# winddori2002/DEX-TTS

Hardware: AMD Instinct MI355X
Metric: mel-frames/s at n_timesteps=50, 80-ch mel (sampler only); RTF (higher is better)
Workload: dtype bf16; 1 GPU; gedex_b1: gedex_lj B=1/GPU T=512 n_timesteps=50 (BASELINE.json configs[1]); global_batch=1, frames=512, hipgraph=False, parallelism=1 GPU

## Files before the change

dex_tts_amd/csrc/dex_api.hip:

```cpp
#include <hip/hip_runtime.h>
#include <cstdlib>

#include <cmath>
#include <cstdarg>
#include <atomic>
#include <cstdio>
#include <mutex>
#include <cstring>
#include <map>
#include <unordered_map>
#include <string_view>
#include <string>
#include <vector>

#include "../../include/dex_amd.h"
#include "kernels.h"
#include "weight_store.h"

using namespace dex;

namespace dex {
namespace {
const char* const KNOB_NAMES[] = {
    "DEX_CONV_STREAM", "DEX_CONV_PP", "DEX_CONV_SKIP_DEAD", "DEX_H_BF16", "DEX_ATTN_SEPARATE", "DEX_ATTN_Q64", "DEX_ATTN_Q64_TAIL", "DEX_ATTN_Q64_HALF", "DEX_DIT_XCDS", "DEX_ATTN_GENERIC", "DEX_RES2", "DEX_LP_INTER", "DEX_DIT_CHAIN",
    "DEX_DIT_CLUSTER", "DEX_DIT_CLUSTER_LOCAL", "DEX_ATTN_X_LP", "DEX_RES_X_LP", "DEX_CAT_LP", "DEX_XCD_MAP", "DEX_DEBUG_DROP_HANDOFF", "DEX_PATCH_FUSED",
    "DEX_CONV_DOWN", "DEX_CONVT_UP", "DEX_DEBUG_PLAN",
    "DEX_ATTN_SHARED_W8", "DEX_CONVT_MT", "DEX_CONVT_WGS", "DEX_CONV_DOWN_WGS", "DEX_CONV_REGW", "DEX_CONV_REGW_RES", "DEX_CONV_SMALL_MAX", "DEX_CONV_TH8",
    "DEX_CONV_W8", "DEX_DWCONV_CAP", "DEX_FINAL_CAP", "DEX_FIRST_CAP", "DEX_FIRST_MFMA", "DEX_GEMM_NWALK", "DEX_NWALK_SPLIT", "DEX_NWALK_BM", "DEX_POS_COL", "DEX_POS_COL_MIN",
    "DEX_POS_CT", "DEX_REGW_MIN_TILES", "DEX_REGW_WGS", "DEX_ROWCHAIN64", "DEX_ROWCHAIN64A", "DEX_TIV_CAP", "DEX_TV_CHAIN", "DEX_TIV_FOLD", "DEX_LINATTN_NSUB", "DEX_TV_FOLD", "DEX_OUT2_MIN", "DEX_NWALK_DMA",
    "DEX_LINATTN_HEADWAVES", "DEX_LINATTN_OUT2_HW", "DEX_CONV_ROUND1", "DEX_CONV_RESIDENT", "DEX_KVCTX_ROWS", "DEX_OUT2_ROWS"};
constexpr int N_KNOBS = (int)(sizeof(KNOB_NAMES) / sizeof(KNOB_NAMES[0]));
int knob_parse(const char* e) {
    if (!e) return KNOB_UNSET;
    char* end = nullptr;
    const long v = strtol(e, &end, 10);
    if (end == e) {
        static bool warned = false;
        if (!warned) { warned = true; fprintf(stderr, "libdexamd: ignoring a DEX_* knob whose value '%s' is not an integer\n", e); }
        return KNOB_UNSET;
    }
    return (int)v;
}
struct KnobSnapshot {
    int v[N_KNOBS];
    KnobSnapshot() { for (int i = 0; i < N_KNOBS; ++i) v[i] = knob_parse(getenv(KNOB_NAMES[i])); }
};
thread_local const KnobSnapshot* t_knobs = nullptr;
struct WsplitScope {
    bool prev;
    explicit WsplitScope(bool on) : prev(g_lp_wsplit) { g_lp_wsplit = on; }
    ~WsplitScope() { g_lp_wsplit = prev; }
};
struct KnobScope {
    const KnobSnapshot* prev;
    explicit KnobScope(const KnobSnapshot* k) : prev(t_knobs) { t_knobs = k; }
    ~KnobScope() { t_knobs = prev; }
};
}
static int knob_index(const char* name) {
    static const std::unordered_map<std::string_view, int> idx = [] {
        std::unordered_map<std::string_view, int> m;
        for (int i = 0; i < N_KNOBS; ++i) m.emplace(KNOB_NAMES[i], i);
        return m;
// ... 1878 lines not shown
```

dex_tts_amd/csrc/igemm_bf16.hip:

```cpp
#include "kernels.h"
#include <cstdlib>
#include "lp_util.h"
#include "kernels_lp.h"
#include "igemm_epilogue.h"

namespace dex {
namespace DEX_LP_NS {

typedef unsigned short u16;


template <int BN, int BK, bool PT, int AP, int RPP, int BP, bool ALP = false>
__device__ __forceinline__ void igemm_load_tile(const IGemmP& p, float4 (&fa)[AP][2], float (&fm)[AP], float (&fo)[AP], uint4& rb0, uint4& rb1,
#ifdef DEX_LP_WSPLIT
                                                uint4& rl0, uint4& rl1,
#endif
                                                int k0, bool live, int tk8, int trow,
                                                const int (&bh)[AP], const int (&bw)[AP], unsigned mvbits,
                                                const float* Ab, const float* mrow, int mws, const u16* Wb, int n0) {
    const int kthr = PT ? k0 + tk8 : k0;
    const int tap = kthr / p.Cin, c0 = kthr - tap * p.Cin + (PT ? 0 : tk8);
    const int kh = tap / p.KW, kw = tap - kh * p.KW;
#pragma unroll
    for (int j = 0; j < AP; ++j) {
// ... 257 lines not shown
                c.z = c.z * rstd * (1.f + sc1.z) + sh1.z; c.w = c.w * rstd * (1.f + sc1.w) + sh1.w;
            }
            const float m_ = mk[j];
            uint4 v;
            v.x = pack2_lp(a.x * m_, a.y * m_); v.y = pack2_lp(a.z * m_, a.w * m_);
            v.z = pack2_lp(c.x * m_, c.y * m_); v.w = pack2_lp(c.z * m_, c.w * m_);
            *reinterpret_cast<uint4*>(As + row * LDS_LD + k8) = v;
        }
    }
    __syncthreads();
    f32x16 acc[MT];
#pragma unroll
    for (int t = 0; t < MT; ++t)
#pragma unroll
        for (int r = 0; r < 16; ++r) acc[t][r] = 0.f;
    const u16* ap = As + (wm * (MT * 32) + i) * LDS_LD + hh * 8;
    const u16* bp = Bs + (wn * 32 + i) * LDS_LD + hh * 8;
#pragma unroll
    for (int ks = 0; ks < K / 16; ++ks) {
        const lp8 bf = *reinterpret_cast<const lp8*>(bp + ks * 16);
#pragma unroll
        for (int t = 0; t < MT; ++t) {
            const lp8 af = *reinterpret_cast<const lp8*>(ap + t * 32 * LDS_LD + ks * 16);
            acc[t] = DEX_MFMA_LP(af, bf, acc[t], 0, 0, 0);
#ifdef DEX_LP_WSPLIT
            acc[t] = DEX_MFMA_LP(af, __builtin_bit_cast(lp8, bl_[ks]), acc[t], 0, 0, 0);
#endif
        }
    }
    igemm_epilogue<MT>(p, acc, m0, n0, wm * (MT * 32), wn * 32, lane, b, 0, 0, M, oh0, ow0);
}

typedef unsigned u32x4 __attribute__((ext_vector_type(4)));
template <int K, int BM = 64, bool DMA = false>
__global__ __launch_bounds__(BM * 4) void igemm_lp_nwalk_kernel(const IGemmP p) {
    constexpr int BN = 64, NTHR = BM * 4;
    constexpr int WN = BN / 32, WM = BM / 32, MT = 1;
    constexpr int LDS_LD = K + 8, KC = K / 8;
    constexpr int AIT = BM * KC / NTHR, BIT = BN * KC / NTHR;
    constexpr int ABATCH = AIT > 8 ? 8 : AIT;
    constexpr int TILE = BN * K;
    static_assert(!DMA || BM == 64, "DMA form: 64-row workgroups");
    extern __shared__ __attribute__((aligned(16))) u16 smem_ss[];
    u16* As = DMA ? smem_ss + TILE : smem_ss;
    u16* Bs = smem_ss + BM * LDS_LD;
    typedef __attribute__((address_space(3))) void* lds_ptr_t;
    const int tid = threadIdx.x, lane = tid & 63, wave = tid >> 6;
    const int i = lane & 31, hh = lane >> 5;
    const int wm = wave / WN, wn = wave % WN;
    const int b = blockIdx.z;
    const int M = p.Ho * p.Wo;
    const int m0 = blockIdx.x * BM;
    const int ntile_all = p.N / BN;
    const int ntile = ntile_all / (int)gridDim.y, nt_first = blockIdx.y * ntile;
    const float* Ab = p.A + (long)b * p.a_bstride + p.a_coff;
    const float* mrow = p.inmask ? p.inmask + (long)b * p.mask_bstride : nullptr;
    const u16* Wb = reinterpret_cast<const u16*>(p.Wbf) + (long)b * p.w_bstride + (long)nt_first * BN * K;
    const int step = p.step + b * p.row_bstride;
    const float* lsh = p.ln_shift ? p.ln_shift + (long)step * p.ln_step_stride : nullptr;
    const float* lsc = p.ln_scale ? p.ln_scale + (long)step * p.ln_step_stride : nullptr;

    const u16* Wf = DMA ? reinterpret_cast<const u16*>(p.Wfrag) + (long)b * p.w_bstride + (long)nt_first * TILE : nullptr;
#define NW_DMA(nt_)                                                                                                 \
    _Pragma("unroll") for (int j = 0; j < 8; ++j) {                                                                \
        const int piece = 8 * wave + j;                                                                             \
        __builtin_amdgcn_global_load_lds(Wf + (long)(nt_) * TILE + piece * 512 + lane * 8,                          \
                                         (lds_ptr_t)(smem_ss + ((nt_) & 1) * TILE + piece * 512), 16, 0, 0);        \
    }
    float* sbias = reinterpret_cast<float*>(smem_ss + TILE + BM * LDS_LD);
    float* smk = sbias + p.N;
    if constexpr (DMA) {
        NW_DMA(0)
        const float* biasg = p.bias ? p.bias + (long)b * p.bias_bstride : nullptr;
        for (int idx = tid; idx < p.N; idx += NTHR) sbias[idx] = biasg ? biasg[idx] : 0.f;
        const float* omg = p.outmask ? p.outmask + (long)b * p.mask_bstride : nullptr;
        const int row = tid >> 2, mrow_ = m0 + row, mm_ = mrow_ < M ? mrow_ : 0, uw_ = (mm_ % p.Wo) * p.unpatch_s;
#pragma unroll
        for (int e = 0; e < 2; ++e) {
            const int sft = (tid & 3) + 4 * e;
            smk[row * 8 + sft] = omg ? omg[min(uw_ + sft, p.OWf - 1) * p.outmask_ws] : 1.f;
        }
    }
    u32x4 br[BIT];
#define NW_LOAD_B(nt_)                                                                                              \
    _Pragma("unroll") for (int j = 0; j < BIT; ++j) {                                                              \
        const int it = tid + NTHR * j;                                                                              \
        br[j] = *reinterpret_cast<const u32x4*>(Wb + (long)((nt_) * BN + it / KC) * K + (it % KC) * 8);            \
    }
#define NW_STORE_B()                                                                                                \
    _Pragma("unroll") for (int j = 0; j < BIT; ++j) {                                                              \
        const int it = tid + NTHR * j;                                                                              \
        *reinterpret_cast<u32x4*>(Bs + (it / KC) * LDS_LD + (it % KC) * 8) = br[j];                                 \
    }
#ifdef DEX_LP_WSPLIT
    const bool has_lo = p.w_lo_off != 0;
    u16* Bl = As;
    u32x4 brl[BIT];
#define NW_LOAD_LO(nt_)                                                                                             \
    _Pragma("unroll") for (int j = 0; j < BIT; ++j) {                                                              \
        const int it = tid + NTHR * j;                                                                              \
        const u32x4 v_ = *reinterpret_cast<const u32x4*>(Wb + (has_lo ? p.w_lo_off : 0) + (long)((nt_) * BN + it / KC) * K + (it % KC) * 8); \
        brl[j] = has_lo ? v_ : u32x4{0u, 0u, 0u, 0u};                                                               \
    }
#define NW_STORE_LO()                                                                                               \
    _Pragma("unroll") for (int j = 0; j < BIT; ++j) {                                                              \
        const int it = tid + NTHR * j;                                                                              \
        *reinterpret_cast<u32x4*>(Bl + (it / KC) * LDS_LD + (it % KC) * 8) = brl[j];                                \
    }
    NW_LOAD_LO(0)
#endif
    if constexpr (!DMA) { NW_LOAD_B(0) }
#pragma unroll
    for (int a0 = 0; a0 < AIT; a0 += ABATCH) {
        float4 f0[ABATCH], f1[ABATCH];
        float mk[ABATCH];
#pragma unroll
        for (int j = 0; j < ABATCH; ++j) {
            const int it = tid + NTHR * (a0 + j);
            const int row = it / KC, k8 = (it % KC) * 8;
            const int m = m0 + row;
            const int mm = m < M ? m : 0;
            const float* src = Ab + (long)mm * p.lda + k8;
            f0[j] = *reinterpret_cast<const float4*>(src);
            f1[j] = *reinterpret_cast<const float4*>(src + 4);
            const float mv = mrow ? mrow[(mm % p.Wi) * p.inmask_ws] : 1.f;
            mk[j] = m < M ? mv : 0.f;
        }
        if constexpr (!DMA) { if (a0 == 0) { NW_STORE_B() } }
#pragma unroll
        for (int j = 0; j < ABATCH; ++j) {
            const int it = tid + NTHR * (a0 + j);
            const int row = it / KC, k8 = (it % KC) * 8;
            float4 a = f0[j], c = f1[j];
            if (lsh) {
                float s = (a.x + a.y) + (a.z + a.w) + (c.x + c.y) + (c.z + c.w);
#pragma unroll
                for (int o = 1; o < KC; o <<= 1) s += __shfl_xor(s, o);
                const float mean = s * (1.f / (float)K);
                a.x -= mean; a.y -= mean; a.z -= mean; a.w -= mean; c.x -= mean; c.y -= mean; c.z -= mean; c.w -= mean;
                float q = a.x * a.x + a.y * a.y + a.z * a.z + a.w * a.w + c.x * c.x + c.y * c.y + c.z * c.z + c.w * c.w;
#pragma unroll
                for (int o = 1; o < KC; o <<= 1) q += __shfl_xor(q, o);
                const float rstd = rsqrtf(q * (1.f / (float)K) + 1e-6f);
                const float4 sc0 = *reinterpret_cast<const float4*>(lsc + k8), sc1 = *reinterpret_cast<const float4*>(lsc + k8 + 4);
                const float4 sh0 = *reinterpret_cast<const float4*>(lsh + k8), sh1 = *reinterpret_cast<const float4*>(lsh + k8 + 4);
                a.x = a.x * rstd * (1.f + sc0.x) + sh0.x; a.y = a.y * rstd * (1.f + sc0.y) + sh0.y;
                a.z = a.z * rstd * (1.f + sc0.z) + sh0.z; a.w = a.w * rstd * (1.f + sc0.w) + sh0.w;
                c.x = c.x * rstd * (1.f + sc1.x) + sh1.x; c.y = c.y * rstd * (1.f + sc1.y) + sh1.y;
                c.z = c.z * rstd * (1.f + sc1.z) + sh1.z; c.w = c.w * rstd * (1.f + sc1.w) + sh1.w;
            }
            const float m_ = mk[j];
            uint4 v;
            v.x = pack2_lp(a.x * m_, a.y * m_); v.y = pack2_lp(a.z * m_, a.w * m_);
            v.z = pack2_lp(c.x * m_, c.y * m_); v.w = pack2_lp(c.z * m_, c.w * m_);
            *reinterpret_cast<uint4*>(As + row * LDS_LD + k8) = v;
        }
    }
    __syncthreads();
    const u16* ap = As + (wm * (MT * 32) + i) * LDS_LD + hh * 8;
    const u16* bp = Bs + (wn * 32 + i) * LDS_LD + hh * 8;
    static_assert(MT == 1, "one 32-row tile per wave");
    lp8 afr[K / 16];
#pragma unroll
    for (int ks = 0; ks < K / 16; ++ks) afr[ks] = *reinterpret_cast<const lp8*>(ap + ks * 16);
#ifdef DEX_LP_WSPLIT
    __syncthreads();
    NW_STORE_LO()
    __syncthreads();
    const u16* blp = Bl + (wn * 32 + i) * LDS_LD + hh * 8;
#endif
    int u_pix, u_f, u_w;
    {
        const int m = m0 + wm * 32 + i;
        const bool v = m < M;
        const int mm = v ? m : 0;
        const int f = mm / p.Wo, w = mm - f * p.Wo;
        u_f = v ? f * p.unpatch_s : 0x40000000;
        u_w = w * p.unpatch_s;
        u_pix = f * p.unpatch_s * p.OWf + w * p.unpatch_s;
    }
    const float* omask = p.outmask ? p.outmask + (long)b * p.mask_bstride : nullptr;
    const float* biasb = p.bias ? p.bias + (long)b * p.bias_bstride : nullptr;
    float4 dst4[4]; char* d_ptr = nullptr; bool d_ok = false, d_all = false, d_have = false;
#define NW_FLUSH()                                                                                                  \
    if (d_have) {                                                                                                   \
        if (p.c_lp) {                                                                                               \
            u16* c_ = reinterpret_cast<u16*>(d_ptr);                                                                \
            if (d_all) { *reinterpret_cast<float4*>(c_) = dst4[0]; *reinterpret_cast<float4*>(c_ + 16) = dst4[1]; } \
            else if (d_ok) { *reinterpret_cast<float4*>(c_) = dst4[0]; *reinterpret_cast<float4*>(c_ + 16) = dst4[1]; } \
        } else {                                                                                                    \
            float* c_ = reinterpret_cast<float*>(d_ptr);                                                            \
// ... 12 lines not shown
#ifdef DEX_LP_WSPLIT
        if (nt + 1 < ntile) { NW_LOAD_LO(nt + 1) }
#endif
        const int ng0 = (nt_first + nt) * BN + wn * 32, pp = ng0 / p.unpatch_C;
        const int u_c0 = ng0 - pp * p.unpatch_C;
        const int u_p1 = pp / p.unpatch_s, u_p2 = pp - u_p1 * p.unpatch_s;
        float u_mk;
        float4 b4[4];
        if constexpr (DMA) {
            u_mk = smk[(wm * 32 + i) * 8 + u_p2];
#pragma unroll
            for (int q = 0; q < 4; ++q) b4[q] = *reinterpret_cast<const float4*>(sbias + ng0 + 8 * q + 4 * hh);
            if (nt + 1 < ntile) { NW_DMA(nt + 1) }
            NW_FLUSH()
        } else {
            u_mk = omask ? omask[min(u_w + u_p2, p.OWf - 1) * p.outmask_ws] : 1.f;
#pragma unroll
            for (int q = 0; q < 4; ++q) b4[q] = biasb ? *reinterpret_cast<const float4*>(biasb + ng0 + 8 * q + 4 * hh) : make_float4(0.f, 0.f, 0.f, 0.f);
        }
        __builtin_amdgcn_sched_barrier(0);
        f32x16 acc[MT];
#pragma unroll
        for (int t = 0; t < MT; ++t)
#pragma unroll
            for (int r = 0; r < 16; ++r) acc[t][r] = 0.f;
#pragma unroll
        for (int ks = 0; ks < K / 16; ++ks) {
            const lp8 bf = *reinterpret_cast<const lp8*>(bp + ks * (DMA ? 512 : 16));
            acc[0] = DEX_MFMA_LP(bf, afr[ks], acc[0], 0, 0, 0);
#ifdef DEX_LP_WSPLIT
            acc[0] = DEX_MFMA_LP(*reinterpret_cast<const lp8*>(blp + ks * 16), afr[ks], acc[0], 0, 0, 0);
#endif
        }
        {
            float val[16];
#pragma unroll
            for (int q = 0; q < 4; ++q) {
                val[4 * q + 0] = (acc[0][4 * q + 0] + b4[q].x) * u_mk; val[4 * q + 1] = (acc[0][4 * q + 1] + b4[q].y) * u_mk;
                val[4 * q + 2] = (acc[0][4 * q + 2] + b4[q].z) * u_mk; val[4 * q + 3] = (acc[0][4 * q + 3] + b4[q].w) * u_mk;
            }
            const bool ok = u_f + u_p1 < p.OHf && u_w + u_p2 < p.OWf;
            const long e0 = (long)b * p.c_bstride + p.c_coff + (long)(u_p1 * p.OWf + u_p2 + u_pix) * p.ldc + u_c0;
            __builtin_amdgcn_sched_barrier(0);
            if (p.c_lp) {
                typedef unsigned u32x2n __attribute__((ext_vector_type(2)));
                unsigned D[4][2];
#pragma unroll
                for (int q = 0; q < 4; ++q) { D[q][0] = pack2_lp(val[4 * q], val[4 * q + 1]); D[q][1] = pack2_lp(val[4 * q + 2], val[4 * q + 3]); }
                uint4 ch[2];
#pragma unroll
                for (int pr = 0; pr < 2; ++pr) {
                    const u32x2n s0 = __builtin_amdgcn_permlane32_swap(D[2 * pr][0], D[2 * pr + 1][0], false, false);
                    const u32x2n s1 = __builtin_amdgcn_permlane32_swap(D[2 * pr][1], D[2 * pr + 1][1], false, false);
                    ch[pr] = make_uint4(s0[0], s1[0], s0[1], s1[1]);
                }
                u16* cph = reinterpret_cast<u16*>(p.C) + e0 + 8 * hh;
                if constexpr (DMA) {
                    dst4[0] = __builtin_bit_cast(float4, ch[0]); dst4[1] = __builtin_bit_cast(float4, ch[1]);
                    d_ptr = reinterpret_cast<char*>(cph); d_ok = ok; d_all = __builtin_amdgcn_ballot_w64(!ok) == 0; d_have = true;
                } else
                if (__builtin_amdgcn_ballot_w64(!ok) == 0) {
                    *reinterpret_cast<uint4*>(cph) = ch[0];
                    *reinterpret_cast<uint4*>(cph + 16) = ch[1];
                } else if (ok) {
                    *reinterpret_cast<uint4*>(cph) = ch[0];
                    *reinterpret_cast<uint4*>(cph + 16) = ch[1];
                }
            } else {
                float* cp = p.C + e0 + 4 * hh;
                if constexpr (DMA) {
#pragma unroll
                    for (int q = 0; q < 4; ++q) dst4[q] = make_float4(val[4 * q], val[4 * q + 1], val[4 * q + 2], val[4 * q + 3]);
                    d_ptr = reinterpret_cast<char*>(cp); d_ok = ok; d_all = __builtin_amdgcn_ballot_w64(!ok) == 0; d_have = true;
                } else
                if (__builtin_amdgcn_ballot_w64(!ok) == 0) {
#pragma unroll
                    for (int q = 0; q < 4; ++q) *reinterpret_cast<float4*>(cp + 8 * q) = make_float4(val[4 * q], val[4 * q + 1], val[4 * q + 2], val[4 * q + 3]);
                } else if (ok) {
#pragma unroll
                    for (int q = 0; q < 4; ++q) *reinterpret_cast<float4*>(cp + 8 * q) = make_float4(val[4 * q], val[4 * q + 1], val[4 * q + 2], val[4 * q + 3]);
                }
            }
        }
        if (!DMA && nt + 1 < ntile) {
            __syncthreads();
            NW_STORE_B()
#ifdef DEX_LP_WSPLIT
            NW_STORE_LO()
#endif
            __syncthreads();
        }
    }
    if constexpr (DMA) { NW_FLUSH() }
}

static bool nwalk_eligible(const IGemmP& p) {
    if (p.a_lp || p.act_in_slope != 0.f) return false;
    if (p.K != 256 || p.Cin != 256 || p.KH != 1 || p.KW != 1 || p.parity || p.ksplit != 1 || p.groups != 1 || (p.N % 64) != 0) return false;
    if (p.sh != 1 || p.sw != 1 || p.off_h != 0 || p.off_w != 0 || p.Ho != p.Hi || p.Wo != p.Wi || p.gn_stats) return false;
    if (p.unpatch_s <= 0 || (p.unpatch_C % 32) != 0 || p.gate || p.res || p.act != 0 || p.stats_final) return false;
    if ((p.ldc % 8) != 0 || (p.c_coff % 8) != 0 || (p.c_bstride % 8) != 0) return false;
    const int mode = knob_or("DEX_GEMM_NWALK", 1);
    if (mode == 0) return false;
    const long wgs = (long)((p.Ho * p.Wo + 63) / 64) * p.B;
    (void)wgs;
    return p.N / 64 >= 8;
}
bool igemm_nwalk_form(const IGemmP& p) {
#if defined(DEX_LP_WSPLIT) && !defined(DEX_WS_HAVE_NWALK)
    return false;
#endif
    return nwalk_eligible(p); }
static void launch_nwalk(const IGemmP& p, hipStream_t st) {
    constexpr int K = 256;
    const size_t lds = (size_t)(64 + 64) * (K + 8) * sizeof(u16), lds128 = (size_t)(128 + 64) * (K + 8) * sizeof(u16);
    static bool attr = false;
    if (!attr) {
        hipFuncSetAttribute(reinterpret_cast<const void*>(&igemm_lp_nwalk_kernel<K>), hipFuncAttributeMaxDynamicSharedMemorySize, (int)lds);
        hipFuncSetAttribute(reinterpret_cast<const void*>(&igemm_lp_nwalk_kernel<K, 128>), hipFuncAttributeMaxDynamicSharedMemorySize, (int)lds128);
#ifndef DEX_LP_WSPLIT
        hipFuncSetAttribute(reinterpret_cast<const void*>(&igemm_lp_nwalk_kernel<K, 64, true>), hipFuncAttributeMaxDynamicSharedMemorySize, 80 * 1024);
#endif
        attr = true;
    }
    {
        const long wgs128 = (long)((p.Ho * p.Wo + 127) / 128) * p.B;
        const int bm_env = knob_or("DEX_NWALK_BM", 0);
        int ns = 1;
        while (ns < 4 && wgs128 * ns < 640 && (p.N / 64) % (ns * 2) == 0) ns *= 2;
        const bool big = bm_env == 128;
        if (big) {
            const int fs = knob_or("DEX_NWALK_SPLIT", 0);
            if (fs > 0 && (p.N / 64) % fs == 0) ns = fs;
            g_last_symbol = "igemm_lp_nwalk_kernel<256, 128>";
            hipLaunchKernelGGL((igemm_lp_nwalk_kernel<K, 128>), dim3((p.Ho * p.Wo + 127) / 128, ns, p.B), dim3(512), lds128, st, p);
            return;
        }
    }
#ifndef DEX_LP_WSPLIT
    if (p.Wfrag && p.w_bstride == 0 && p.N <= 2048 && p.unpatch_s <= 8 && knob_or("DEX_NWALK_DMA", 0) != 0) {
        const size_t lds_dma = (size_t)64 * K * 2 + (size_t)64 * (K + 8) * 2 + (size_t)p.N * 4 + 64 * 8 * 4;
        const long wgs = (long)((p.Ho * p.Wo + 63) / 64) * p.B;
        int nsplit = 1;
        const int fs = knob_or("DEX_NWALK_SPLIT", 0);
        while (nsplit < 4 && wgs * nsplit < 1280 && (p.N / 64) % (nsplit * 2) == 0) nsplit *= 2;
        if (wgs <= 16) nsplit = p.N / 64;
        if (fs > 0 && (p.N / 64) % fs == 0) nsplit = fs;
        g_last_symbol = "igemm_lp_nwalk_kernel<256,64,1>";
        hipLaunchKernelGGL((igemm_lp_nwalk_kernel<K, 64, true>), dim3((p.Ho * p.Wo + 63) / 64, nsplit, p.B), dim3(256), lds_dma, st, p);
        return;
    }
#endif
    g_last_symbol = "igemm_lp_nwalk_kernel<256>";
    const long wgs = (long)((p.Ho * p.Wo + 63) / 64) * p.B;
    int nsplit = 1;
    const int fs = knob_or("DEX_NWALK_SPLIT", 0);
    while (nsplit < 4 && wgs * nsplit < 1280 && (p.N / 64) % (nsplit * 2) == 0) nsplit *= 2;
    if (wgs <= 16) nsplit = p.N / 64;
    if (fs > 0 && (p.N / 64) % fs == 0) nsplit = fs;
    dim3 grid((p.Ho * p.Wo + 63) / 64, nsplit, p.B);
    hipLaunchKernelGGL((igemm_lp_nwalk_kernel<K>), grid, dim3(256), lds, st, p);
}

template <int K>
static void launch_ss(const IGemmP& p, hipStream_t st) {
    const size_t lds = (size_t)(64 + 64) * (K + 8) * sizeof(u16);
    static bool attr = false;
    if (!attr) {
        hipFuncSetAttribute(reinterpret_cast<const void*>(&igemm_lp_ss_kernel<64, 64, K>), hipFuncAttributeMaxDynamicSharedMemorySize, (int)lds);
        hipFuncSetAttribute(reinterpret_cast<const void*>(&igemm_lp_ss_kernel<64, 64, K, true>), hipFuncAttributeMaxDynamicSharedMemorySize, (int)lds);
        attr = true;
    }
    dim3 grid((p.Ho * p.Wo + 63) / 64, p.N / 64, p.B * (p.parity ? 4 : 1));
    if (p.a_lp) hipLaunchKernelGGL((igemm_lp_ss_kernel<64, 64, K, true>), grid, dim3(256), lds, st, p);
    else hipLaunchKernelGGL((igemm_lp_ss_kernel<64, 64, K>), grid, dim3(256), lds, st, p);
}

static bool ss_eligible(const IGemmP& p) {
    if (p.c_lp || p.act_in_slope != 0.f) return false;
    if (p.a_lp && (p.ln_shift || p.KH != 1 || p.KW != 1 || (p.Cin % 8) != 0)) return false;
    if (p.ksplit != 1 || p.groups != 1 || (p.N % 64) != 0) return false;
    if (p.K != 64 && p.K != 128 && p.K != 256 && p.K != 512) return false;
    const long blocks = (long)((p.Ho * p.Wo + 63) / 64) * (p.N / 64) * p.B;
// ... 65 lines not shown
```

dex_tts_amd/csrc/patch_embed.hip:

```cpp
#include <hip/hip_runtime.h>
#include "kernels.h"
#include "lp_util.h"
#include "kernels_lp.h"

namespace dex {
namespace DEX_LP_NS {

typedef float f32x16 __attribute__((ext_vector_type(16)));
typedef unsigned short u16;

namespace {
constexpr int PE_TOK = 8;
__device__ __forceinline__ float silu_pe(float x) { return x * __builtin_amdgcn_rcpf(1.f + __expf(-x)); }
}

template <int KS, int C>
__global__ __launch_bounds__(256) void patch_embed_fused_kernel(const DwConvP p, const u16* __restrict__ Wb, const float* __restrict__ bias, float* __restrict__ emb, int hid) {
    constexpr int C4 = C / 4, LD = C + 8, KSTEPS = C / 16;
    constexpr int IPT = PE_TOK * C4 / 256;
    __shared__ __attribute__((aligned(16))) u16 As[32 * LD];
    const int tid = threadIdx.x, lane = tid & 63, wave = tid >> 6;
    const int i = lane & 31, hh = lane >> 5;
    const long ntok = (long)p.B * p.Hf * p.Wt;
    const long tok0 = (long)blockIdx.x * PE_TOK;
    const int ntile = hid / 32, per_wave = ntile / 4;
    union Fr { uint4 u; lp8 v; };
    Fr wf[2][KSTEPS];
#ifdef DEX_LP_WSPLIT
    Fr wl[2][KSTEPS];
#endif
    auto wload_tile = [&](int slot, int nt) __attribute__((always_inline)) {
        const u16* src = Wb + (long)(nt * 32 + i) * C + hh * 8;
#pragma unroll
        for (int ks = 0; ks < KSTEPS; ++ks) wf[slot][ks].u = *reinterpret_cast<const uint4*>(src + ks * 16);
    };
    auto wload_lo = [&](int slot, int nt) __attribute__((always_inline)) {
#ifdef DEX_LP_WSPLIT
        const u16* src = Wb + (long)hid * C + (long)(nt * 32 + i) * C + hh * 8;
#pragma unroll
        for (int ks = 0; ks < KSTEPS; ++ks) wl[slot][ks].u = *reinterpret_cast<const uint4*>(src + ks * 16);
#endif
    };
    wload_tile(0, wave * per_wave);
    if (per_wave > 1) wload_tile(1, wave * per_wave + 1);
    for (int q = tid; q < (32 - PE_TOK) * LD / 8; q += 256) *reinterpret_cast<uint4*>(As + PE_TOK * LD + q * 8) = make_uint4(0, 0, 0, 0);
    if (tid < PE_TOK * C4) {
        const int cq = tid % C4, tl = tid / C4;
        const long tok = min(tok0 + tl, ntok - 1);
        const int wt = (int)(tok % p.Wt);
        const int f = (int)((tok / p.Wt) % p.Hf);
        const int b = (int)(tok / ((long)p.Wt * p.Hf));
        const float* X = p.X + (long)b * p.xb;
        const float* mrow = p.mask ? p.mask + (long)b * p.mask_bstride : nullptr;
        float4 acc = *reinterpret_cast<const float4*>(p.bd + cq * 4);
        const float4 a4 = p.aff ? *reinterpret_cast<const float4*>(p.aff + ((long)b * 2 + 0) * p.C + cq * 4) : make_float4(1.f, 1.f, 1.f, 1.f);
        const float4 c4 = p.aff ? *reinterpret_cast<const float4*>(p.aff + ((long)b * 2 + 1) * p.C + cq * 4) : make_float4(0.f, 0.f, 0.f, 0.f);
#pragma unroll
        for (int kh = 0; kh < KS; ++kh) {
            const int hi = f * p.s + kh - p.pad;
#pragma unroll
            for (int kw = 0; kw < KS; ++kw) {
                const int wi = wt * p.s + kw - p.pad;
                const bool inb = (unsigned)hi < (unsigned)p.Hi && (unsigned)wi < (unsigned)p.Wi;
                const int hc = inb ? hi : 0, wc = inb ? wi : 0;
                float4 v = *reinterpret_cast<const float4*>(X + ((long)hc * p.Wi + wc) * p.ldx + cq * 4);
                if (p.aff) { v.x = fmaf(v.x, a4.x, c4.x); v.y = fmaf(v.y, a4.y, c4.y); v.z = fmaf(v.z, a4.z, c4.z); v.w = fmaf(v.w, a4.w, c4.w); }
                const float4 w = *reinterpret_cast<const float4*>(p.Wd + (kh * KS + kw) * p.C + cq * 4);
                float mk = mrow ? mrow[wc * p.mask_ws] : 1.f;
                mk = inb ? mk : 0.f;
                acc.x = fmaf(v.x * mk, w.x, acc.x); acc.y = fmaf(v.y * mk, w.y, acc.y);
                acc.z = fmaf(v.z * mk, w.z, acc.z); acc.w = fmaf(v.w * mk, w.w, acc.w);
            }
        }
        uint2 o;
        o.x = pack2_lp(silu_pe(acc.x), silu_pe(acc.y)); o.y = pack2_lp(silu_pe(acc.z), silu_pe(acc.w));
        *reinterpret_cast<uint2*>(As + tl * LD + cq * 4) = o;
    }
    wload_lo(0, wave * per_wave);
    if (per_wave > 1) wload_lo(1, wave * per_wave + 1);
    __syncthreads();
    const u16* a_lane = As + i * LD + hh * 8;
    for (int t0 = 0; t0 < per_wave; t0 += 2) {
#pragma unroll
        for (int s_ = 0; s_ < 2; ++s_) {
            if (t0 + s_ >= per_wave) break;
            const int nt = wave * per_wave + t0 + s_;
            f32x16 acc;
#pragma unroll
            for (int r = 0; r < 16; ++r) acc[r] = 0.f;
#pragma unroll
            for (int ks = 0; ks < KSTEPS; ++ks) {
                const lp8 af = *reinterpret_cast<const lp8*>(a_lane + ks * 16);
                acc = DEX_MFMA_LP(af, wf[s_][ks].v, acc, 0, 0, 0);
#ifdef DEX_LP_WSPLIT
                acc = DEX_MFMA_LP(af, wl[s_][ks].v, acc, 0, 0, 0);
#endif
            }
            const float bv = bias ? bias[nt * 32 + i] : 0.f;
#pragma unroll
            for (int r = 0; r < 4; ++r) {
                const int rowl = r + 4 * hh;
                if (tok0 + rowl < ntok) emb[(tok0 + rowl) * hid + nt * 32 + i] = acc[r] + bv;
            }
        }
        if (t0 + 2 < per_wave) {
            wload_tile(0, wave * per_wave + t0 + 2); wload_lo(0, wave * per_wave + t0 + 2);
            if (t0 + 3 < per_wave) { wload_tile(1, wave * per_wave + t0 + 3); wload_lo(1, wave * per_wave + t0 + 3); }
        }
    }
}

bool patch_embed_fused_supported(int k, int C, int hid, long ntok) {
#if defined(DEX_LP_WSPLIT) && !defined(DEX_WS_HAVE_PE)
    return false;
#endif
   
    return (k == 3 || k == 7) && (C == 64 || C == 128) && hid % 128 == 0 && (ntok * (C / 4) + 255) / 256 < 320;
}

void launch_patch_embed_fused(const DwConvP& p, const void* Wb, const float* bias, float* emb, int hid, hipStream_t st) {
    const long ntok = (long)p.B * p.Hf * p.Wt;
    const dim3 grid((unsigned)((ntok + PE_TOK - 1) / PE_TOK));
    const u16* w = reinterpret_cast<const u16*>(Wb);
    g_last_symbol = "patch_embed_fused_kernel";
    if (p.k == 7 && p.C == 128) hipLaunchKernelGGL((patch_embed_fused_kernel<7, 128>), grid, dim3(256), 0, st, p, w, bias, emb, hid);
    else if (p.k == 7) hipLaunchKernelGGL((patch_embed_fused_kernel<7, 64>), grid, dim3(256), 0, st, p, w, bias, emb, hid);
    else if (p.C == 128) hipLaunchKernelGGL((patch_embed_fused_kernel<3, 128>), grid, dim3(256), 0, st, p, w, bias, emb, hid);
    else hipLaunchKernelGGL((patch_embed_fused_kernel<3, 64>), grid, dim3(256), 0, st, p, w, bias, emb, hid);
}

}
}
```

Baseline: 29030 mel-frames/s.

## Add small-batch variants for patch-embed and n-walk GEMM to fill more CUs

Adds a patch-embed kernel variant that handles fewer tokens per workgroup (4 or 2), so a small token count spreads over more CUs. This variant stages the depthwise weights in shared memory using spare waves and prefetches its inputs into registers. Adds an n-walk GEMM variant with 32-row workgroups, where each wave keeps its own 64-column weight fragments in registers, chosen by a heuristic for small batches. The aim is better occupancy at B=1; the cost is redundant weight loads per workgroup and extra timing instrumentation compiled in only under DEX_TIMING.

```diff
diff --git a/dex_tts_amd/csrc/dex_api.hip b/dex_tts_amd/csrc/dex_api.hip
--- a/dex_tts_amd/csrc/dex_api.hip
+++ b/dex_tts_amd/csrc/dex_api.hip
@@ -28,7 +28,7 @@
     "DEX_ATTN_SHARED_W8", "DEX_CONVT_MT", "DEX_CONVT_WGS", "DEX_CONV_DOWN_WGS", "DEX_CONV_REGW", "DEX_CONV_REGW_RES", "DEX_CONV_SMALL_MAX", "DEX_CONV_TH8",
     "DEX_CONV_W8", "DEX_DWCONV_CAP", "DEX_FINAL_CAP", "DEX_FIRST_CAP", "DEX_FIRST_MFMA", "DEX_GEMM_NWALK", "DEX_NWALK_SPLIT", "DEX_NWALK_BM", "DEX_POS_COL", "DEX_POS_COL_MIN",
     "DEX_POS_CT", "DEX_REGW_MIN_TILES", "DEX_REGW_WGS", "DEX_ROWCHAIN64", "DEX_ROWCHAIN64A", "DEX_TIV_CAP", "DEX_TV_CHAIN", "DEX_TIV_FOLD", "DEX_LINATTN_NSUB", "DEX_TV_FOLD", "DEX_OUT2_MIN", "DEX_NWALK_DMA",
-    "DEX_LINATTN_HEADWAVES", "DEX_LINATTN_OUT2_HW", "DEX_CONV_ROUND1", "DEX_CONV_RESIDENT", "DEX_KVCTX_ROWS", "DEX_OUT2_ROWS"};
+    "DEX_LINATTN_HEADWAVES", "DEX_LINATTN_OUT2_HW", "DEX_CONV_ROUND1", "DEX_CONV_RESIDENT", "DEX_KVCTX_ROWS", "DEX_OUT2_ROWS", "DEX_PE_TOK", "DEX_NWALK_SMALL"};
 constexpr int N_KNOBS = (int)(sizeof(KNOB_NAMES) / sizeof(KNOB_NAMES[0]));
 int knob_parse(const char* e) {
     if (!e) return KNOB_UNSET;
diff --git a/dex_tts_amd/csrc/igemm_bf16.hip b/dex_tts_amd/csrc/igemm_bf16.hip
--- a/dex_tts_amd/csrc/igemm_bf16.hip
+++ b/dex_tts_amd/csrc/igemm_bf16.hip
@@ -313,6 +313,21 @@
 }
 
 typedef unsigned u32x4 __attribute__((ext_vector_type(4)));
+#ifdef DEX_TIMING
+__device__ long long* nw_dbg = nullptr;
+void nw_set_dbg(long long* d) { (void)hipMemcpyToSymbol(HIP_SYMBOL(nw_dbg), &d, sizeof d); }
+#define NSTAMP_DECL long long tk[8] = {0, 0, 0, 0, 0, 0, 0, 0}; const long long tk0 = __builtin_readcyclecounter(); long long tlast = tk0;
+#define NSTAMP(k) do { const long long now_ = __builtin_readcyclecounter(); tk[k] += now_ - tlast; tlast = now_; } while (0)
+#define NSTAMP_STORE()                                                                                                \
+    if (nw_dbg && threadIdx.x == 0) {                                                                                 \
+        tk[7] = __builtin_readcyclecounter() - tk0;                                                                   \
+        for (int k_ = 0; k_ < 8; ++k_) nw_dbg[((long)blockIdx.y * gridDim.x + blockIdx.x) * 8 + k_] = tk[k_];         \
+    }
+#else
+#define NSTAMP_DECL
+#define NSTAMP(k) do {} while (0)
+#define NSTAMP_STORE()
+#endif
 template <int K, int BM = 64, bool DMA = false>
 __global__ __launch_bounds__(BM * 4) void igemm_lp_nwalk_kernel(const IGemmP p) {
     constexpr int BN = 64, NTHR = BM * 4;
@@ -332,6 +347,7 @@
     const int b = blockIdx.z;
     const int M = p.Ho * p.Wo;
     const int m0 = blockIdx.x * BM;
+    NSTAMP_DECL
     const int ntile_all = p.N / BN;
     const int ntile = ntile_all / (int)gridDim.y, nt_first = blockIdx.y * ntile;
     const float* Ab = p.A + (long)b * p.a_bstride + p.a_coff;
@@ -391,6 +407,7 @@
     NW_LOAD_LO(0)
 #endif
     if constexpr (!DMA) { NW_LOAD_B(0) }
+    NSTAMP(0);
 #pragma unroll
     for (int a0 = 0; a0 < AIT; a0 += ABATCH) {
         float4 f0[ABATCH], f1[ABATCH];
@@ -437,7 +454,9 @@
             *reinterpret_cast<uint4*>(As + row * LDS_LD + k8) = v;
         }
     }
+    NSTAMP(1);
     __syncthreads();
+    NSTAMP(2);
     const u16* ap = As + (wm * (MT * 32) + i) * LDS_LD + hh * 8;
     const u16* bp = Bs + (wn * 32 + i) * LDS_LD + hh * 8;
     static_assert(MT == 1, "one 32-row tile per wave");
@@ -516,6 +535,7 @@
             acc[0] = DEX_MFMA_LP(*reinterpret_cast<const lp8*>(blp + ks * 16), afr[ks], acc[0], 0, 0, 0);
 #endif
         }
+        NSTAMP(3);
         {
             float val[16];
 #pragma unroll
@@ -566,6 +586,7 @@
                 }
             }
         }
+        NSTAMP(4);
         if (!DMA && nt + 1 < ntile) {
             __syncthreads();
             NW_STORE_B()
@@ -576,6 +597,151 @@
         }
     }
     if constexpr (DMA) { NW_FLUSH() }
+    NSTAMP_STORE()
+}
+
+template <int K>
+__global__ __launch_bounds__(256) void igemm_lp_nwalk_kernel_small(const IGemmP p) {
+    constexpr int BM = 32, NTHR = 256, LDS_LD = K + 8, KC = K / 8, AIT = BM * KC / NTHR;
+    static_assert(KC == 32 && AIT * NTHR == BM * KC, "a row = 32 lanes of 8 values");
+    __shared__ __attribute__((aligned(16))) u16 As[BM * LDS_LD];
+    const int tid = threadIdx.x, lane = tid & 63, wave = tid >> 6;
+    const int i = lane & 31, hh = lane >> 5;
+    const int b = blockIdx.z;
+    const int M = p.Ho * p.Wo;
+    const int m0 = blockIdx.x * BM;
+    const int ct = blockIdx.y * 4 + wave;
+    NSTAMP_DECL
+    const float* Ab = p.A + (long)b * p.a_bstride + p.a_coff;
+    const float* mrow = p.inmask ? p.inmask + (long)b * p.mask_bstride : nullptr;
+    const int step = p.step + b * p.row_bstride;
+    const float* lsh = p.ln_shift ? p.ln_shift + (long)step * p.ln_step_stride : nullptr;
+    const float* lsc = p.ln_scale ? p.ln_scale + (long)step * p.ln_step_stride : nullptr;
+    const int k8 = (tid % KC) * 8;
+    float4 f0[AIT], f1[AIT];
+    float mk[AIT];
+#pragma unroll
+    for (int j = 0; j < AIT; ++j) {
+        const int row = (tid + NTHR * j) / KC;
+        const int m = m0 + row;
+        const int mm = m < M ? m : 0;
+        const float* src = Ab + (long)mm * p.lda + k8;
+        f0[j] = *reinterpret_cast<const float4*>(src);
+        f1[j] = *reinterpret_cast<const float4*>(src + 4);
+        const float mv = mrow ? mrow[(mm % p.Wi) * p.inmask_ws] : 1.f;
+        mk[j] = m < M ? mv : 0.f;
+    }
+    float4 sc0 = make_float4(0.f, 0.f, 0.f, 0.f), sc1 = sc0, sh0 = sc0, sh1 = sc0;
+    if (lsh) {
+        sc0 = *reinterpret_cast<const float4*>(lsc + k8); sc1 = *reinterpret_cast<const float4*>(lsc + k8 + 4);
+        sh0 = *reinterpret_cast<const float4*>(lsh + k8); sh1 = *reinterpret_cast<const float4*>(lsh + k8 + 4);
+    }
+    union Fr { uint4 u; lp8 v; };
+    Fr wfr[2][K / 16];
+    {
+        const uint4* Wf = reinterpret_cast<const uint4*>(p.Wfrag) + (long)ct * (2 * (K / 16) * 64) + lane;
+#pragma unroll
+        for (int wn = 0; wn < 2; ++wn)
+#pragma unroll
+            for (int ks = 0; ks < K / 16; ++ks) wfr[wn][ks].u = Wf[(wn * (K / 16) + ks) * 64];
+    }
+    NSTAMP(0);
+#pragma unroll
+    for (int j = 0; j < AIT; ++j) {
+        const int row = (tid + NTHR * j) / KC;
+        float4 a = f0[j], c = f1[j];
+        if (lsh) {
+            float s = (a.x + a.y) + (a.z + a.w) + (c.x + c.y) + (c.z + c.w);
+#pragma unroll
+            for (int o = 1; o < KC; o <<= 1) s += __shfl_xor(s, o);
+            const float mean = s * (1.f / (float)K);
+            a.x -= mean; a.y -= mean; a.z -= mean; a.w -= mean; c.x -= mean; c.y -= mean; c.z -= mean; c.w -= mean;
+            float q = a.x * a.x + a.y * a.y + a.z * a.z + a.w * a.w + c.x * c.x + c.y * c.y + c.z * c.z + c.w * c.w;
+#pragma unroll
+            for (int o = 1; o < KC; o <<= 1) q += __shfl_xor(q, o);
+            const float rstd = rsqrtf(q * (1.f / (float)K) + 1e-6f);
+            a.x = a.x * rstd * (1.f + sc0.x) + sh0.x; a.y = a.y * rstd * (1.f + sc0.y) + sh0.y;
+            a.z = a.z * rstd * (1.f + sc0.z) + sh0.z; a.w = a.w * rstd * (1.f + sc0.w) + sh0.w;
+            c.x = c.x * rstd * (1.f + sc1.x) + sh1.x; c.y = c.y * rstd * (1.f + sc1.y) + sh1.y;
+            c.z = c.z * rstd * (1.f + sc1.z) + sh1.z; c.w = c.w * rstd * (1.f + sc1.w) + sh1.w;
+        }
+        const float m_ = mk[j];
+        uint4 v;
+        v.x = pack2_lp(a.x * m_, a.y * m_); v.y = pack2_lp(a.z * m_, a.w * m_);
+        v.z = pack2_lp(c.x * m_, c.y * m_); v.w = pack2_lp(c.z * m_, c.w * m_);
+        *reinterpret_cast<uint4*>(As + row * LDS_LD + k8) = v;
+    }
+    NSTAMP(1);
+    lds_barrier();
+    NSTAMP(2);
+    lp8 afr[K / 16];
+    {
+        const u16* ap = As + i * LDS_LD + hh * 8;
+#pragma unroll
+        for (int ks = 0; ks < K / 16; ++ks) afr[ks] = *reinterpret_cast<const lp8*>(ap + ks * 16);
+    }
+    int u_pix, u_f, u_w;
+    {
+        const int m = m0 + i;
+        const bool v = m < M;
+        const int mm = v ? m : 0;
+        const int f = mm / p.Wo, w = mm - f * p.Wo;
+        u_f = v ? f * p.unpatch_s : 0x40000000;
+        u_w = w * p.unpatch_s;
+        u_pix = f * p.unpatch_s * p.OWf + w * p.unpatch_s;
+    }
+    const float* omask = p.outmask ? p.outmask + (long)b * p.mask_bstride : nullptr;
+    const float* biasb = p.bias ? p.bias + (long)b * p.bias_bstride : nullptr;
+#pragma unroll
+    for (int wn = 0; wn < 2; ++wn) {
+        const int ng0 = ct * 64 + wn * 32, pp = ng0 / p.unpatch_C;
+        const int u_c0 = ng0 - pp * p.unpatch_C;
+        const int u_p1 = pp / p.unpatch_s, u_p2 = pp - u_p1 * p.unpatch_s;
+        const float u_mk = omask ? omask[min(u_w + u_p2, p.OWf - 1) * p.outmask_ws] : 1.f;
+        float4 b4[4];
+#pragma unroll
+        for (int q = 0; q < 4; ++q) b4[q] = biasb ? *reinterpret_cast<const float4*>(biasb + ng0 + 8 * q + 4 * hh) : make_float4(0.f, 0.f, 0.f, 0.f);
+        f32x16 acc;
+#pragma unroll
+        for (int r = 0; r < 16; ++r) acc[r] = 0.f;
+#pragma unroll
+        for (int ks = 0; ks < K / 16; ++ks) acc = DEX_MFMA_LP(wfr[wn][ks].v, afr[ks], acc, 0, 0, 0);
+        NSTAMP(3);
+        float val[16];
+#pragma unroll
+        for (int q = 0; q < 4; ++q) {
+            val[4 * q + 0] = (acc[4 * q + 0] + b4[q].x) * u_mk; val[4 * q + 1] = (acc[4 * q + 1] + b4[q].y) * u_mk;
+            val[4 * q + 2] = (acc[4 * q + 2] + b4[q].z) * u_mk; val[4 * q + 3] = (acc[4 * q + 3] + b4[q].w) * u_mk;
+        }
+        const bool ok = u_f + u_p1 < p.OHf && u_w + u_p2 < p.OWf;
+        const long e0 = (long)b * p.c_bstride + p.c_coff + (long)(u_p1 * p.OWf + u_p2 + u_pix) * p.ldc + u_c0;
+        if (p.c_lp) {
+            typedef unsigned u32x2n __attribute__((ext_vector_type(2)));
+            unsigned D[4][2];
+#pragma unroll
+            for (int q = 0; q < 4; ++q) { D[q][0] = pack2_lp(val[4 * q], val[4 * q + 1]); D[q][1] = pack2_lp(val[4 * q + 2], val[4 * q + 3]); }
+            uint4 ch[2];
+#pragma unroll
+            for (int pr = 0; pr < 2; ++pr) {
+                const u32x2n s0 = __builtin_amdgcn_permlane32_swap(D[2 * pr][0], D[2 * pr + 1][0], false, false);
+                const u32x2n s1 = __builtin_amdgcn_permlane32_swap(D[2 * pr][1], D[2 * pr + 1][1], false, false);
+                ch[pr] = make_uint4(s0[0], s1[0], s0[1], s1[1]);
+            }
+            u16* cph = reinterpret_cast<u16*>(p.C) + e0 + 8 * hh;
+            if (ok) {
+                *reinterpret_cast<uint4*>(cph) = ch[0];
+                *reinterpret_cast<uint4*>(cph + 16) = ch[1];
+            }
+        } else {
+            float* cp = p.C + e0 + 4 * hh;
+            if (ok) {
+#pragma unroll
+                for (int q = 0; q < 4; ++q) *reinterpret_cast<float4*>(cp + 8 * q) = make_float4(val[4 * q], val[4 * q + 1], val[4 * q + 2], val[4 * q + 3]);
+            }
+        }
+        NSTAMP(4);
+    }
+    NSTAMP_STORE()
 }
 
 static bool nwalk_eligible(const IGemmP& p) {
@@ -633,6 +799,19 @@
         g_last_symbol = "igemm_lp_nwalk_kernel<256,64,1>";
         hipLaunchKernelGGL((igemm_lp_nwalk_kernel<K, 64, true>), dim3((p.Ho * p.Wo + 63) / 64, nsplit, p.B), dim3(256), lds_dma, st, p);
         return;
+    }
+#endif
+#ifndef DEX_LP_WSPLIT
+    if (p.Wfrag && p.w_bstride == 0 && (p.N % 256) == 0 && knob_or("DEX_NWALK_SPLIT", 0) <= 0) {
+        const int rt64 = (p.Ho * p.Wo + 63) / 64, rt32 = (p.Ho * p.Wo + 31) / 32;
+        const long ncu = device_cus();
+        const bool rule = p.B < 4 && (long)rt64 * p.B <= 16 && (long)rt64 * p.B * (p.N / 64) > ncu && (long)rt32 * p.B * (p.N / 256) <= ncu;
+        const int mode = knob_or("DEX_NWALK_SMALL", -1);
+        if (mode > 0 || (mode < 0 && rule)) {
+            g_last_symbol = "igemm_lp_nwalk_kernel_small<256>";
+            hipLaunchKernelGGL((igemm_lp_nwalk_kernel_small<K>), dim3(rt32, p.N / 256, p.B), dim3(256), 0, st, p);
+            return;
+        }
     }
 #endif
     g_last_symbol = "igemm_lp_nwalk_kernel<256>";
diff --git a/dex_tts_amd/csrc/patch_embed.hip b/dex_tts_amd/csrc/patch_embed.hip
--- a/dex_tts_amd/csrc/patch_embed.hip
+++ b/dex_tts_amd/csrc/patch_embed.hip
@@ -8,21 +8,47 @@
 
 typedef float f32x16 __attribute__((ext_vector_type(16)));
 typedef unsigned short u16;
+typedef float f32x4 __attribute__((ext_vector_type(4)));
+
+#ifdef DEX_TIMING
+__device__ long long* pe_dbg = nullptr;
+void pe_set_dbg(long long* d) { (void)hipMemcpyToSymbol(HIP_SYMBOL(pe_dbg), &d, sizeof d); }
+#define PSTAMP_DECL long long tk[8] = {0, 0, 0, 0, 0, 0, 0, 0}; const long long tk0 = __builtin_readcyclecounter(); long long tlast = tk0;
+#define PSTAMP(k) do { const long long now_ = __builtin_readcyclecounter(); tk[k] += now_ - tlast; tlast = now_; } while (0)
+#define PSTAMP_STORE()                                                                                                \
+    if (pe_dbg && threadIdx.x == 0) {                                                                                 \
+        tk[7] = __builtin_readcyclecounter() - tk0;                                                                   \
+        for (int k_ = 0; k_ < 8; ++k_) pe_dbg[(long)blockIdx.x * 8 + k_] = tk[k_];                                    \
+    }
+__device__ int pe_cut = 0;
+static int pe_cut_host = 0;
+void pe_set_cut(int n) { pe_cut_host = n; (void)hipMemcpyToSymbol(HIP_SYMBOL(pe_cut), &n, sizeof n); }
+#define PE_LIVE(TOK) ((TOK) == PE_TOK && pe_cut > 0 ? pe_cut : (TOK))
+#define PE_LIVE_HOST(TOK) ((TOK) == PE_TOK && pe_cut_host > 0 ? pe_cut_host : (TOK))
+#else
+#define PSTAMP_DECL
+#define PSTAMP(k) do {} while (0)
+#define PSTAMP_STORE()
+#define PE_LIVE(TOK) (TOK)
+#define PE_LIVE_HOST(TOK) (TOK)
+#endif
 
 namespace {
 constexpr int PE_TOK = 8;
+constexpr int PE_TOK_MIN = 4;
 __device__ __forceinline__ float silu_pe(float x) { return x * __builtin_amdgcn_rcpf(1.f + __expf(-x)); }
 }
 
-template <int KS, int C>
+template <int KS, int C, int TOK = PE_TOK>
 __global__ __launch_bounds__(256) void patch_embed_fused_kernel(const DwConvP p, const u16* __restrict__ Wb, const float* __restrict__ bias, float* __restrict__ emb, int hid) {
     constexpr int C4 = C / 4, LD = C + 8, KSTEPS = C / 16;
-    constexpr int IPT = PE_TOK * C4 / 256;
+    static_assert(TOK == 8 || TOK == 4 || TOK == 2, "tokens per workgroup");
     __shared__ __attribute__((aligned(16))) u16 As[32 * LD];
     const int tid = threadIdx.x, lane = tid & 63, wave = tid >> 6;
     const int i = lane & 31, hh = lane >> 5;
+    PSTAMP_DECL
     const long ntok = (long)p.B * p.Hf * p.Wt;
-    const long tok0 = (long)blockIdx.x * PE_TOK;
+    const long tok0 = (long)blockIdx.x * PE_LIVE(TOK);
     const int ntile = hid / 32, per_wave = ntile / 4;
     union Fr { uint4 u; lp8 v; };
     Fr wf[2][KSTEPS];
@@ -43,8 +69,12 @@
     };
     wload_tile(0, wave * per_wave);
     if (per_wave > 1) wload_tile(1, wave * per_wave + 1);
-    for (int q = tid; q < (32 - PE_TOK) * LD / 8; q += 256) *reinterpret_cast<uint4*>(As + PE_TOK * LD + q * 8) = make_uint4(0, 0, 0, 0);
-    if (tid < PE_TOK * C4) {
+    for (int q = tid; q < (32 - TOK) * LD / 8; q += 256) *reinterpret_cast<uint4*>(As + TOK * LD + q * 8) = make_uint4(0, 0, 0, 0);
+    if constexpr (TOK != PE_TOK) {
+        __shared__ __attribute__((aligned(16))) float Wds[KS * KS * C];
+        constexpr int NW4 = KS * KS * C4, DWW = (TOK * C4 + 63) / 64, NST = 256 - DWW * 64, WIT = (NW4 + NST - 1) / NST;
+        static_assert(DWW <= 2, "at least two waves stage the weights");
+        const bool dw = tid < TOK * C4;
         const int cq = tid % C4, tl = tid / C4;
         const long tok = min(tok0 + tl, ntok - 1);
         const int wt = (int)(tok % p.Wt);
@@ -52,33 +82,104 @@
         const int b = (int)(tok / ((long)p.Wt * p.Hf));
         const float* X = p.X + (long)b * p.xb;
         const float* mrow = p.mask ? p.mask + (long)b * p.mask_bstride : nullptr;
-        float4 acc = *reinterpret_cast<const float4*>(p.bd + cq * 4);
-        const float4 a4 = p.aff ? *reinterpret_cast<const float4*>(p.aff + ((long)b * 2 + 0) * p.C + cq * 4) : make_float4(1.f, 1.f, 1.f, 1.f);
-        const float4 c4 = p.aff ? *reinterpret_cast<const float4*>(p.aff + ((long)b * 2 + 1) * p.C + cq * 4) : make_float4(0.f, 0.f, 0.f, 0.f);
-#pragma unroll
-        for (int kh = 0; kh < KS; ++kh) {
-            const int hi = f * p.s + kh - p.pad;
+        float4 acc = make_float4(0.f, 0.f, 0.f, 0.f), a4 = make_float4(1.f, 1.f, 1.f, 1.f), c4 = acc;
+        float mkc[KS];
+        f32x4 xv[KS * KS];
+        if (dw) {
+            acc = *reinterpret_cast<const float4*>(p.bd + cq * 4);
+            if (p.aff) {
+                a4 = *reinterpret_cast<const float4*>(p.aff + ((long)b * 2 + 0) * p.C + cq * 4);
+                c4 = *reinterpret_cast<const float4*>(p.aff + ((long)b * 2 + 1) * p.C + cq * 4);
+            }
 #pragma unroll
             for (int kw = 0; kw < KS; ++kw) {
                 const int wi = wt * p.s + kw - p.pad;
-                const bool inb = (unsigned)hi < (unsigned)p.Hi && (unsigned)wi < (unsigned)p.Wi;
-                const int hc = inb ? hi : 0, wc = inb ? wi : 0;
-                float4 v = *reinterpret_cast<const float4*>(X + ((long)hc * p.Wi + wc) * p.ldx + cq * 4);
-                if (p.aff) { v.x = fmaf(v.x, a4.x, c4.x); v.y = fmaf(v.y, a4.y, c4.y); v.z = fmaf(v.z, a4.z, c4.z); v.w = fmaf(v.w, a4.w, c4.w); }
-                const float4 w = *reinterpret_cast<const float4*>(p.Wd + (kh * KS + kw) * p.C + cq * 4);
-                float mk = mrow ? mrow[wc * p.mask_ws] : 1.f;
-                mk = inb ? mk : 0.f;
-                acc.x = fmaf(v.x * mk, w.x, acc.x); acc.y = fmaf(v.y * mk, w.y, acc.y);
-                acc.z = fmaf(v.z * mk, w.z, acc.z); acc.w = fmaf(v.w * mk, w.w, acc.w);
-            }
-        }
-        uint2 o;
-        o.x = pack2_lp(silu_pe(acc.x), silu_pe(acc.y)); o.y = pack2_lp(silu_pe(acc.z), silu_pe(acc.w));
-        *reinterpret_cast<uint2*>(As + tl * LD + cq * 4) = o;
-    }
+                const int wcc = (unsigned)wi < (unsigned)p.Wi ? wi : 0;
+                mkc[kw] = mrow ? mrow[wcc * p.mask_ws] : 1.f;
+            }
+#pragma unroll
+            for (int kh = 0; kh < KS; ++kh) {
+                const int hi = f * p.s + kh - p.pad;
+#pragma unroll
+                for (int kw = 0; kw < KS; ++kw) {
+                    const int wi = wt * p.s + kw - p.pad;
+                    const bool inb = (unsigned)hi < (unsigned)p.Hi && (unsigned)wi < (unsigned)p.Wi;
+                    const int hc = inb ? hi : 0, wc = inb ? wi : 0;
+                    xv[kh * KS + kw] = *reinterpret_cast<const f32x4*>(X + ((long)hc * p.Wi + wc) * p.ldx + cq * 4);
+                }
+            }
+        }
+        if (wave >= DWW) {
+            const int t0 = tid - DWW * 64;
+            f32x4 ws[WIT];
+#pragma unroll
+            for (int j = 0; j < WIT; ++j) ws[j] = *reinterpret_cast<const f32x4*>(p.Wd + min(t0 + NST * j, NW4 - 1) * 4);
+#pragma unroll
+            for (int j = 0; j < WIT; ++j)
+                if (t0 + NST * j < NW4) *reinterpret_cast<f32x4*>(Wds + (t0 + NST * j) * 4) = ws[j];
+        }
+        PSTAMP(0);
+        lds_barrier();
+        PSTAMP(1);
+        if (dw) {
+#pragma unroll
+            for (int kh = 0; kh < KS; ++kh) {
+                const int hi = f * p.s + kh - p.pad;
+#pragma unroll
+                for (int kw = 0; kw < KS; ++kw) {
+                    const int wi = wt * p.s + kw - p.pad;
+                    const bool inb = (unsigned)hi < (unsigned)p.Hi && (unsigned)wi < (unsigned)p.Wi;
+                    f32x4 v = xv[kh * KS + kw];
+                    if (p.aff) { v.x = fmaf(v.x, a4.x, c4.x); v.y = fmaf(v.y, a4.y, c4.y); v.z = fmaf(v.z, a4.z, c4.z); v.w = fmaf(v.w, a4.w, c4.w); }
+                    const float4 w = *reinterpret_cast<const float4*>(Wds + (kh * KS + kw) * C + cq * 4);
+                    const float mk = inb ? mkc[kw] : 0.f;
+                    acc.x = fmaf(v.x * mk, w.x, acc.x); acc.y = fmaf(v.y * mk, w.y, acc.y);
+                    acc.z = fmaf(v.z * mk, w.z, acc.z); acc.w = fmaf(v.w * mk, w.w, acc.w);
+                }
+            }
+            uint2 o;
+            o.x = pack2_lp(silu_pe(acc.x), silu_pe(acc.y)); o.y = pack2_lp(silu_pe(acc.z), silu_pe(acc.w));
+            *reinterpret_cast<uint2*>(As + tl * LD + cq * 4) = o;
+        }
+    } else {
+        if (tid < PE_LIVE(TOK) * C4) {
+            const int cq = tid % C4, tl = tid / C4;
+            const long tok = min(tok0 + tl, ntok - 1);
+            const int wt = (int)(tok % p.Wt);
+            const int f = (int)((tok / p.Wt) % p.Hf);
+            const int b = (int)(tok / ((long)p.Wt * p.Hf));
+            const float* X = p.X + (long)b * p.xb;
+            const float* mrow = p.mask ? p.mask + (long)b * p.mask_bstride : nullptr;
+            float4 acc = *reinterpret_cast<const float4*>(p.bd + cq * 4);
+            const float4 a4 = p.aff ? *reinterpret_cast<const float4*>(p.aff + ((long)b * 2 + 0) * p.C + cq * 4) : make_float4(1.f, 1.f, 1.f, 1.f);
+            const float4 c4 = p.aff ? *reinterpret_cast<const float4*>(p.aff + ((long)b * 2 + 1) * p.C + cq * 4) : make_float4(0.f, 0.f, 0.f, 0.f);
+#pragma unroll
+            for (int kh = 0; kh < KS; ++kh) {
+                const int hi = f * p.s + kh - p.pad;
+#pragma unroll
+                for (int kw = 0; kw < KS; ++kw) {
+                    const int wi = wt * p.s + kw - p.pad;
+                    const bool inb = (unsigned)hi < (unsigned)p.Hi && (unsigned)wi < (unsigned)p.Wi;
+                    const int hc = inb ? hi : 0, wc = inb ? wi : 0;
+                    float4 v = *reinterpret_cast<const float4*>(X + ((long)hc * p.Wi + wc) * p.ldx + cq * 4);
+                    if (p.aff) { v.x = fmaf(v.x, a4.x, c4.x); v.y = fmaf(v.y, a4.y, c4.y); v.z = fmaf(v.z, a4.z, c4.z); v.w = fmaf(v.w, a4.w, c4.w); }
+                    const float4 w = *reinterpret_cast<const float4*>(p.Wd + (kh * KS + kw) * p.C + cq * 4);
+                    float mk = mrow ? mrow[wc * p.mask_ws] : 1.f;
+                    mk = inb ? mk : 0.f;
+                    acc.x = fmaf(v.x * mk, w.x, acc.x); acc.y = fmaf(v.y * mk, w.y, acc.y);
+                    acc.z = fmaf(v.z * mk, w.z, acc.z); acc.w = fmaf(v.w * mk, w.w, acc.w);
+                }
+            }
+            uint2 o;
+            o.x = pack2_lp(silu_pe(acc.x), silu_pe(acc.y)); o.y = pack2_lp(silu_pe(acc.z), silu_pe(acc.w));
+            *reinterpret_cast<uint2*>(As + tl * LD + cq * 4) = o;
+        }
+    }
+    PSTAMP(2);
     wload_lo(0, wave * per_wave);
     if (per_wave > 1) wload_lo(1, wave * per_wave + 1);
     __syncthreads();
+    PSTAMP(3);
     const u16* a_lane = As + i * LD + hh * 8;
     for (int t0 = 0; t0 < per_wave; t0 += 2) {
 #pragma unroll
@@ -96,11 +197,12 @@
                 acc = DEX_MFMA_LP(af, wl[s_][ks].v, acc, 0, 0, 0);
 #endif
             }
+            PSTAMP(4);
             const float bv = bias ? bias[nt * 32 + i] : 0.f;
 #pragma unroll
             for (int r = 0; r < 4; ++r) {
                 const int rowl = r + 4 * hh;
-                if (tok0 + rowl < ntok) emb[(tok0 + rowl) * hid + nt * 32 + i] = acc[r] + bv;
+                if (rowl < PE_LIVE(TOK) && tok0 + rowl < ntok) emb[(tok0 + rowl) * hid + nt * 32 + i] = acc[r] + bv;
             }
         }
         if (t0 + 2 < per_wave) {
@@ -108,6 +210,8 @@
             if (t0 + 3 < per_wave) { wload_tile(1, wave * per_wave + t0 + 3); wload_lo(1, wave * per_wave + t0 + 3); }
         }
     }
+    PSTAMP(5);
+    PSTAMP_STORE()
 }
 
 bool patch_embed_fused_supported(int k, int C, int hid, long ntok) {
@@ -118,16 +222,34 @@
     return (k == 3 || k == 7) && (C == 64 || C == 128) && hid % 128 == 0 && (ntok * (C / 4) + 255) / 256 < 320;
 }
 
+template <int TOK>
+static void pe_launch(const DwConvP& p, const u16* w, const float* bias, float* emb, int hid, long ntok, hipStream_t st) {
+    const dim3 grid((unsigned)((ntok + PE_LIVE_HOST(TOK) - 1) / PE_LIVE_HOST(TOK)));
+    if (p.k == 7 && p.C == 128) hipLaunchKernelGGL((patch_embed_fused_kernel<7, 128, TOK>), grid, dim3(256), 0, st, p, w, bias, emb, hid);
+    else if (p.k == 7) hipLaunchKernelGGL((patch_embed_fused_kernel<7, 64, TOK>), grid, dim3(256), 0, st, p, w, bias, emb, hid);
+    else if (p.C == 128) hipLaunchKernelGGL((patch_embed_fused_kernel<3, 128, TOK>), grid, dim3(256), 0, st, p, w, bias, emb, hid);
+    else hipLaunchKernelGGL((patch_embed_fused_kernel<3, 64, TOK>), grid, dim3(256), 0, st, p, w, bias, emb, hid);
+}
+
+static int pe_tokens(long ntok, int B) {
+    const int forced = knob_or("DEX_PE_TOK", 0);
+    if (forced == 2 || forced == 4 || forced == 8) return forced;
+    const long ncu = device_cus();
+    if (B >= 4) return PE_TOK;
+    for (int t = PE_TOK_MIN; t < PE_TOK; t *= 2)
+        if ((ntok + t - 1) / t <= ncu) return t;
+    return PE_TOK;
+}
+
 void launch_patch_embed_fused(const DwConvP& p, const void* Wb, const float* bias, float* emb, int hid, hipStream_t st) {
     const long ntok = (long)p.B * p.Hf * p.Wt;
-    const dim3 grid((unsigned)((ntok + PE_TOK - 1) / PE_TOK));
     const u16* w = reinterpret_cast<const u16*>(Wb);
-    g_last_symbol = "patch_embed_fused_kernel";
-    if (p.k == 7 && p.C == 128) hipLaunchKernelGGL((patch_embed_fused_kernel<7, 128>), grid, dim3(256), 0, st, p, w, bias, emb, hid);
-    else if (p.k == 7) hipLaunchKernelGGL((patch_embed_fused_kernel<7, 64>), grid, dim3(256), 0, st, p, w, bias, emb, hid);
-    else if (p.C == 128) hipLaunchKernelGGL((patch_embed_fused_kernel<3, 128>), grid, dim3(256), 0, st, p, w, bias, emb, hid);
-    else hipLaunchKernelGGL((patch_embed_fused_kernel<3, 64>), grid, dim3(256), 0, st, p, w, bias, emb, hid);
-}
-
-}
-}
+    switch (pe_tokens(ntok, p.B)) {
+    case 2: g_last_symbol = "patch_embed_fused_kernel<2>"; pe_launch<2>(p, w, bias, emb, hid, ntok, st); break;
+    case 4: g_last_symbol = "patch_embed_fused_kernel<4>"; pe_launch<4>(p, w, bias, emb, hid, ntok, st); break;
+    default: g_last_symbol = "patch_embed_fused_kernel"; pe_launch<PE_TOK>(p, w, bias, emb, hid, ntok, st); break;
+    }
+}
+
+}
+}
```

Result: faster. 29650 mel-frames/s (median of 6 runs) (+2.1%).
